# DavidPetrus/ood_object_detection

Measured on AMD Instinct MI355X. Metric: images/sec, tf_efficientdet_d0 640px bf16 inference + OOD score (DetBenchPredict end-to-end), higher is better.
Workload: dtype bf16; 1 GPU; tf_efficientdet_d0 640x640 batch=64/GPU C=90, DetBenchPredict: backbone+BiFPN+heads+OOD energy/max-logit+top-k(5000)+decode+hard NMS; global_batch=64, parallelism=image-sharded dp1, no collective, weights=seeded reference init, randomised BN stats, class bias 0, launch=hipgraph, images_in_flight=192

## Files before the change

### include/effdet_hip.h

```cpp
#ifndef EFFDET_HIP_H
#define EFFDET_HIP_H

#ifdef __cplusplus
extern "C" {
#endif

#define EFFDET_F32 0
#define EFFDET_BF16 1
#define EFFDET_BF16X2 2
#define EFFDET_PAD_SYMMETRIC (1 << 24)

int effdet_abi_version(void);
const char* effdet_last_error(void);
int effdet_device_error(int clear);


int effdet_stem_conv(void* stream, int in_dtype, int out_dtype, const void* X, const float* Wt,
                     const float* scale, const float* shift, void* Y, int B, int H, int W, int Cout);

int effdet_stem_dw_fused(void* stream, int in_dtype, int dtype, const void* X, const void* Wk,
                         const float* s1, const float* t1, const float* taps, const float* s2, const float* t2,
                         void* Y, float* pool_partial, int B, int H, int W, int C);
int effdet_stem_dw_parts(int dtype, int H, int W, int C);
#define EFFDET_STEM_DW_PLAN_INTS 13
int effdet_stem_dw_plan_describe(int dtype, int in_dtype, int H, int W, int C, int* out, int n);

int effdet_resize_pad_u8(void* stream, const unsigned char* src, int h, int w, unsigned char* dst, int S, int sw, int sh,
                         const int* bounds_x, const int* coef_x, int ksize_x,
                         const int* bounds_y, const int* coef_y, int ksize_y,
                         const int* fill_rgb, unsigned char* workspace);
int effdet_normalize_u8(void* stream, int out_dtype, const unsigned char* X, const float* mean, const float* stdv,
                        void* Y, int B, int C, long long hw);

typedef struct EffdetResampleDesc {
    const unsigned char* src;
    int h, w;
    int flip_h, flip_v;
    int cx0, cy0, cw, ch;
    int filter;
    int sw, sh;
    int ox, oy;
    int reserved;
} EffdetResampleDesc;
int effdet_resample_batch_u8(void* stream, const EffdetResampleDesc* desc, const EffdetResampleDesc* desc_host, int B,
                             unsigned char* dst, long long dst_image_stride, int S, const int* fill_rgb);

typedef struct EffdetBoxParams {
    float img_w, img_h;
    int flip_h, flip_v;
    float pre_y, pre_x, scale, post_y, post_x, clip_h, clip_w;
    int reserved;
} EffdetBoxParams;
int effdet_transform_boxes(void* stream, const float* boxes, const long long* classes, const EffdetBoxParams* params,
                           int B, int Mmax, float* out_boxes, long long* out_classes, int* counts, unsigned char* valid);
int effdet_stem_conv_u8(void* stream, int out_dtype, const unsigned char* X, const float* mean, const float* stdv,
                        const float* Wt, const float* scale, const float* shift, void* Y, int B, int H, int W, int Cout);
int effdet_stem_dw_fused_u8(void* stream, int dtype, const unsigned char* X, const float* mean, const float* stdv,
                            const void* Wk, const float* s1, const float* t1, const float* taps, const float* s2, const float* t2,
                            void* Y, float* pool_partial, int B, int H, int W, int C);

int effdet_pw_gemm_bn_act(void* stream, int dtype, const void* A, long long M, int K, const void* W, int N,
                          const float* scale, const float* shift, int act, const void* residual,
                          const float* gate, int rows_per_image,
                          void* C, long long c_image_stride, long long ldc);
int effdet_pw_gemm_group(void* stream, int dtype, int n, const void* const* A, const long long* M, const int* K,
                         const void* const* W, const int* N, const float* const* scale, const float* const* shift,
                         int act, void* const* C);
#define EFFDET_PW_GEMM_PLAN_INTS 13
int effdet_pw_gemm_plan_describe(int dtype, long long M, int K, int N, int rows_per_image, int gated, int has_residual,
                                 long long ldc, long long c_image_stride, int aligned, int group, int* out, int n);
int effdet_pw_gemm_group_plan_describe(int dtype, int n_problems, const long long* M, const int* K, const int* N, int aligned,
                                       int which, int* out, int n);

int effdet_dwconv_bn_act(void* stream, int dtype, const void* X, void* Y, const float* Wt,
                         const float* scale, const float* shift, int act, float* pool_partial,
                         int B, int H, int W, int C, int k, int stride);
int effdet_dwconv_blocks_per_image(int Ho, int Wo, int C);
#define EFFDET_DWCONV_PLAN_INTS 10
int effdet_dwconv_plan_describe(int dtype, int H, int W, int C, int k, int stride, int pooled, int* out, int n);

int effdet_mbconv_expand_dw(void* stream, int dtype, const void* X, void* Y, const void* W1,
                            const float* s1, const float* t1, const float* taps,
                            const float* s2, const float* t2, float* pool_partial,
                            int B, int H, int W, int Cin, int mid, int k, int stride);
int effdet_mbconv_tiles_per_image(int dtype, int H, int W, int Cin, int mid, int k, int stride);
int effdet_mbconv_expand_dw_gated(void* stream, int dtype, const void* X, const float* in_gate, void* Y, const void* W1,
                                  const float* s1, const float* t1, const float* taps,
                                  const float* s2, const float* t2, float* pool_partial,
                                  int B, int H, int W, int Cin, int mid, int k, int stride);
int effdet_mbconv_gated_tiles_per_image(int dtype, int H, int W, int Cin, int mid, int k, int stride);
#define EFFDET_MBCONV_PLAN_INTS 17
int effdet_mbconv_plan_describe(int dtype, int H, int W, int Cin, int mid, int k, int stride, int gated, int* out, int n);

int effdet_se_gate(void* stream, const float* partial, int nblk, int hw, const float* W1, const float* b1,
                   const float* W2t, const float* b2, float* gate, int B, int C, int R);


int effdet_maxpool_same(void* stream, int dtype, const void* X, long long x_image_stride,
                        void* Y, long long y_image_stride, int B, int H, int W, int C);

int effdet_sepconv_fused(void* stream, int dtype, int B, int nlevels, const int* level_hw, int n_in,
                         const void* const* in_ptr, const long long* in_image_stride, const int* in_hw,
                         const int* in_mode, int fuse_mode, const float* fuse_w, float fuse_den, int pre_act,
                         const float* dw_w, const void* pw_w, const float* scale, const float* shift,
                         const int* affine_row, int post_act, int F, int N,
                         void* const* out_ptr, const long long* out_image_stride,
                         int ood_classes, int num_anchors, float* ood_energy, float* ood_maxlogit,
                         long long ood_image_stride, const long long* ood_level_off);
#define EFFDET_SEPCONV_PLAN_INTS 18
int effdet_sepconv_plan_describe(int dtype, int nlevels, const int* level_hw, int n_in, int F, int N, int ood_classes,
                                 int num_anchors, int has_scale, int post_act, int aligned, int* out, int n);

int effdet_sepconv_meta(void* stream, int dtype, int B, int nlevels, const int* level_hw,
                        const void* const* in_ptr, const long long* in_image_stride,
                        const float* in_scale, const float* in_shift, const int* in_affine_row, int pre_act,
                        const float* dw_w, const void* pw_w, const float* bias, int F, int N,
                        void* const* out_ptr, const long long* out_image_stride,
                        float* stat_partial, void* const* dw_out, const long long* dw_out_image_stride);
int effdet_sepconv_tiles(int dtype, int nlevels, const int* level_hw, int* level_tile_begin);
int effdet_bn_batch_stats(void* stream, int dtype, const float* partial, int B, int nlevels, const int* level_hw, int N,
                          const float* weight, const float* bias, const int* param_row, float eps,
                          float* out_scale, float* out_shift);


long long effdet_topk_workspace_bytes(int B, long long n_anchors);
// ... 466 lines not shown
```

### ood_object_detection_amd/_lib.py

```python
import ctypes
import os
import subprocess

_HERE = os.path.dirname(os.path.abspath(__file__))
LIB_PATH = os.path.join(_HERE, 'libeffdet_hip.so')
CSRC = os.path.join(_HERE, 'csrc')

_lib = None

LABEL_PAD = -2 ** 63

c_void_p, c_int, c_ll, c_float, c_double = ctypes.c_void_p, ctypes.c_int, ctypes.c_longlong, ctypes.c_float, ctypes.c_double
P = ctypes.POINTER

SIGNATURES = {
    'effdet_abi_version': (c_int, []),
    'effdet_last_error': (ctypes.c_char_p, []),
    'effdet_device_error': (c_int, [c_int]),
    'effdet_stem_conv': (c_int, [c_void_p, c_int, c_int, c_void_p, c_void_p, c_void_p, c_void_p, c_void_p,
                                 c_int, c_int, c_int, c_int]),
    'effdet_stem_dw_fused': (c_int, [c_void_p, c_int, c_int, c_void_p, c_void_p, c_void_p, c_void_p, c_void_p, c_void_p,
                                     c_void_p, c_void_p, c_void_p, c_int, c_int, c_int, c_int]),
    'effdet_resize_pad_u8': (c_int, [c_void_p, c_void_p, c_int, c_int, c_void_p, c_int, c_int, c_int, c_void_p, c_void_p, c_int,
                                     c_void_p, c_void_p, c_int, c_void_p, c_void_p]),
    'effdet_resample_batch_u8': (c_int, [c_void_p, c_void_p, c_void_p, c_int, c_void_p, c_ll, c_int, c_void_p]),
    'effdet_transform_boxes': (c_int, [c_void_p, c_void_p, c_void_p, c_void_p, c_int, c_int, c_void_p, c_void_p, c_void_p, c_void_p]),
    'effdet_normalize_u8': (c_int, [c_void_p, c_int, c_void_p, c_void_p, c_void_p, c_void_p, c_int, c_int, c_ll]),
    'effdet_stem_conv_u8': (c_int, [c_void_p, c_int, c_void_p, c_void_p, c_void_p, c_void_p, c_void_p, c_void_p, c_void_p,
                                    c_int, c_int, c_int, c_int]),
    'effdet_stem_dw_fused_u8': (c_int, [c_void_p, c_int, c_void_p, c_void_p, c_void_p, c_void_p, c_void_p, c_void_p, c_void_p,
                                        c_void_p, c_void_p, c_void_p, c_void_p, c_int, c_int, c_int, c_int]),
    'effdet_stem_dw_parts': (c_int, [c_int, c_int, c_int, c_int]),
    'effdet_stem_dw_plan_describe': (c_int, [c_int, c_int, c_int, c_int, c_int, P(c_int), c_int]),
    'effdet_pw_gemm_bn_act': (c_int, [c_void_p, c_int, c_void_p, c_ll, c_int, c_void_p, c_int, c_void_p, c_void_p,
                                      c_int, c_void_p, c_void_p, c_int, c_void_p, c_ll, c_ll]),
    'effdet_pw_gemm_group': (c_int, [c_void_p, c_int, c_int, P(c_void_p), P(c_ll), P(c_int), P(c_void_p), P(c_int), P(c_void_p),
                                     P(c_void_p), c_int, P(c_void_p)]),
    'effdet_dwconv_bn_act': (c_int, [c_void_p, c_int, c_void_p, c_void_p, c_void_p, c_void_p, c_void_p, c_int,
                                     c_void_p, c_int, c_int, c_int, c_int, c_int, c_int]),
    'effdet_dwconv_blocks_per_image': (c_int, [c_int, c_int, c_int]),
    'effdet_dwconv_plan_describe': (c_int, [c_int, c_int, c_int, c_int, c_int, c_int, c_int, P(c_int), c_int]),
    'effdet_pw_gemm_plan_describe': (c_int, [c_int, c_ll, c_int, c_int, c_int, c_int, c_int, c_ll, c_ll, c_int, c_int, P(c_int), c_int]),
    'effdet_pw_gemm_group_plan_describe': (c_int, [c_int, c_int, P(c_ll), P(c_int), P(c_int), c_int, c_int, P(c_int), c_int]),
    'effdet_mbconv_gated_tiles_per_image': (c_int, [c_int, c_int, c_int, c_int, c_int, c_int, c_int]),
    'effdet_mbconv_expand_dw_gated': (c_int, [c_void_p, c_int, c_void_p, c_void_p, c_void_p, c_void_p, c_void_p, c_void_p, c_void_p,
                                              c_void_p, c_void_p, c_void_p, c_int, c_int, c_int, c_int, c_int, c_int, c_int]),
    'effdet_mbconv_expand_dw': (c_int, [c_void_p, c_int, c_void_p, c_void_p, c_void_p, c_void_p, c_void_p, c_void_p,
                                        c_void_p, c_void_p, c_void_p, c_int, c_int, c_int, c_int, c_int, c_int, c_int]),
    'effdet_mbconv_tiles_per_image': (c_int, [c_int, c_int, c_int, c_int, c_int, c_int, c_int]),
    'effdet_mbconv_plan_describe': (c_int, [c_int, c_int, c_int, c_int, c_int, c_int, c_int, c_int, P(c_int), c_int]),
    'effdet_se_gate': (c_int, [c_void_p, c_void_p, c_int, c_int, c_void_p, c_void_p, c_void_p, c_void_p,
                               c_void_p, c_int, c_int, c_int]),
    'effdet_maxpool_same': (c_int, [c_void_p, c_int, c_void_p, c_ll, c_void_p, c_ll, c_int, c_int, c_int, c_int]),
    'effdet_sepconv_fused': (c_int, [c_void_p, c_int, c_int, c_int, P(c_int), c_int,
                                     P(c_void_p), P(c_ll), P(c_int), P(c_int), c_int, P(c_float), c_float, c_int,
                                     c_void_p, c_void_p, c_void_p, c_void_p, P(c_int), c_int, c_int, c_int,
                                     P(c_void_p), P(c_ll), c_int, c_int, c_void_p, c_void_p, c_ll, P(c_ll)]),
    'effdet_sepconv_plan_describe': (c_int, [c_int, c_int, P(c_int), c_int, c_int, c_int, c_int, c_int, c_int, c_int, c_int, P(c_int), c_int]),
    'effdet_weighted_median': (c_int, [c_void_p, c_void_p, c_void_p, c_int, c_int, c_void_p, c_void_p]),
    'effdet_sqnorm_workspace_floats': (c_ll, []),
    'effdet_sqnorm': (c_int, [c_void_p, c_void_p, c_ll, c_void_p, c_void_p, c_int]),
    'effdet_adam_clip_step': (c_int, [c_void_p, c_void_p, c_void_p, c_void_p, c_void_p, c_ll, c_float, c_float, c_float, c_float,
                                      c_int, c_float, c_void_p]),
    'effdet_adam_clip_step_dev': (c_int, [c_void_p, c_void_p, c_void_p, c_void_p, c_void_p, c_ll, c_float, c_float, c_float, c_float,
                                          c_void_p, c_float, c_void_p]),
    'effdet_group_piece_floats': (c_ll, []),
    'effdet_group_norms': (c_int, [c_void_p, c_void_p, c_ll, c_void_p, c_int, c_int, c_void_p, c_int, c_void_p, c_int, c_void_p, c_int,
                                   c_void_p, c_void_p]),
    'effdet_group_step': (c_int, [c_void_p, c_int, c_void_p, c_void_p, c_void_p, c_void_p, c_ll, c_void_p, c_int, c_int, c_void_p, c_int,
                                  c_void_p, c_int, c_void_p, c_int, c_void_p, c_void_p, c_void_p, c_void_p]),
    'effdet_novelty_score': (c_int, [c_void_p, c_void_p, c_void_p, c_void_p, c_int, c_int, c_int, c_float, c_float, c_int,
                                     c_void_p, c_void_p, c_void_p]),
    'effdet_ood_image_score': (c_int, [c_void_p, c_void_p, c_int, c_ll, c_void_p]),
    'effdet_auroc_counts': (c_int, [c_void_p, c_void_p, c_void_p, c_int, c_int, c_void_p]),
    'effdet_ood_eval_workspace_bytes': (c_ll, [c_ll, c_ll]),
    'effdet_ood_eval_sort_tile': (c_int, []),
    'effdet_ood_eval_sorted_offset': (c_ll, [c_ll, c_ll, c_int]),
    'effdet_ood_eval_append': (c_int, [c_void_p, c_void_p, c_ll, c_ll, c_int, c_int, c_void_p, c_int, c_void_p, c_ll, c_ll, c_float,
                                       c_int, c_void_p, c_ll, c_void_p, c_void_p, c_ll]),
    'effdet_ood_eval_sort': (c_int, [c_void_p, c_void_p, c_ll, c_void_p, c_ll, c_void_p, c_void_p, c_ll]),
    'effdet_ood_eval_metrics': (c_int, [c_void_p, c_ll, c_ll, c_void_p, c_void_p, c_ll, c_double, c_void_p]),
    'effdet_feature_ood_workspace_bytes': (c_ll, [c_ll, c_int]),
    'effdet_feature_ood_fit': (c_int, [c_void_p, c_int, c_int, P(c_void_p), P(c_ll), P(c_ll), P(c_ll), P(c_ll), c_int, c_int, c_int, c_int,
                                       c_ll, c_void_p, c_void_p, c_int, c_ll, c_ll, c_ll, c_void_p, c_int, c_void_p, c_void_p, c_void_p,
                                       c_void_p, c_ll]),
    'effdet_feature_ood_score': (c_int, [c_void_p, c_int, c_int, P(c_void_p), P(c_ll), P(c_ll), P(c_ll), P(c_ll), c_int, c_int, c_int,
                                         c_int, c_ll, c_void_p, c_void_p, c_int, c_void_p, c_void_p, c_void_p, c_void_p, c_void_p,
                                         c_void_p, c_void_p, c_void_p]),
    'effdet_feature_knn_workspace_bytes': (c_ll, [c_ll, c_int, c_int, c_int]),
    'effdet_feature_knn_append': (c_int, [c_void_p, c_int, c_int, P(c_void_p), P(c_ll), P(c_ll), P(c_ll), P(c_ll), c_int, c_int, c_int, c_int,
                                          c_ll, c_void_p, c_void_p, c_int, c_ll, c_ll, c_ll, c_void_p, c_int, c_int, c_ll, c_ll, c_void_p,
                                          c_void_p, c_void_p, c_void_p, c_void_p, c_ll]),
    'effdet_feature_knn_score': (c_int, [c_void_p, c_int, c_int, P(c_void_p), P(c_ll), P(c_ll), P(c_ll), P(c_ll), c_int, c_int, c_int,
                                         c_ll, c_void_p, c_void_p, c_int, c_int, c_int, c_int, c_ll, c_void_p, c_void_p, c_void_p,
                                         c_void_p, c_void_p, c_void_p, c_void_p, c_ll]),
    'effdet_feature_subspace_score': (c_int, [c_void_p, c_int, c_int, P(c_void_p), P(c_ll), P(c_ll), P(c_ll), P(c_ll), c_int, c_int, c_int,
# ... 278 lines not shown
```

### ood_object_detection_amd/csrc/pw_gemm.hip

```cpp
#include "common.h"

namespace {

struct PwArgs {
    const void* A; long long M; int K;
    const void* W; int N;
    const float* scale; const float* shift; int act;
    const void* res;
    const float* gate; int rows_per_image;
    void* C; long long c_image_stride; long long ldc;
    int tiles_per_image, n_tiles, vec_ok;
};

template <int V> struct PwInt { static constexpr int value = V; };

constexpr int PW_PIX = 128;

template <typename T, int BN> struct PwGeom {
    static constexpr int KCH = IsPair<T>::value ? 1 : 2;
    static constexpr int ROWB = KCH * OpGeom<T>::CHUNK + 16;
    static constexpr int W_BYTES = BN * ROWB;
    static constexpr int LDS_BYTES = 2 * W_BYTES;
    __host__ __device__ static inline int chunks(int K) { return (K + OpGeom<T>::KPC - 1) / OpGeom<T>::KPC; }
    __host__ __device__ static inline int stages(int K) { return (chunks(K) + KCH - 1) / KCH; }
};

template <typename T, int BN, int PT, int NTH, bool GATED>
DEV void pw_gemm_body(const PwArgs& p, const int bid) {
    constexpr bool PAIR = IsPair<T>::value;
    constexpr int KCH = PwGeom<T, BN>::KCH;
    constexpr int EPC = VecTraits<T>::EPC;
    constexpr int KPC = OpGeom<T>::KPC;
    constexpr int PB = OpGeom<T>::PIECE, CB = OpGeom<T>::CHUNK;
    constexpr int NT = BN / 16, NP = NT / 2;
    static_assert(NT % 2 == 0, "tile pairs");
    constexpr int PF = 2;
    constexpr int ROWB = PwGeom<T, BN>::ROWB;
    constexpr int W_BYTES = PwGeom<T, BN>::W_BYTES;
    static_assert(ROWB == KCH * CB + 16, "one stage of K + 16 pad");
    __shared__ __attribute__((aligned(16))) char lds[PwGeom<T, BN>::LDS_BYTES];
    extern __shared__ __attribute__((aligned(16))) float gate_lds[];

    const int tid = threadIdx.x, lane = tid & 63, wave = tid >> 6;
    const int frow = lane & 15, fpiece = lane >> 4;
    const int K = p.K, N = p.N;
    const int nt = bid % p.n_tiles;
    const int mt = bid / p.n_tiles;
    const int img = mt / p.tiles_per_image;
    const int pix0 = (mt - img * p.tiles_per_image) * PW_PIX;
    const int n0 = nt * BN;
    const int n_count = (N - n0) < BN ? (N - n0) : BN;
    const long long pitch = (long long)K * (long long)sizeof(T);
    const int nst = PwGeom<T, BN>::stages(K);
// ... 277 lines not shown
        default: return EFFDET_EINVAL;
    }
#undef PW_LAUNCH
#undef PW_LAUNCH_G
#undef PW_FORM
    return plan ? EFFDET_OK : effdet_check_launch();
}

int pw_single(hipStream_t st, int dtype, PwArgs& a, PwPlan* plan) {
    if (!a.A || !a.W || !a.C || !a.shift || a.M <= 0 || a.K <= 0 || a.N <= 0) return EFFDET_EINVAL;
    if (a.K % 8 != 0 || a.M > 0x7fffffffLL) return EFFDET_EINVAL;
    if (a.act < 0 || a.act > 2) return EFFDET_EINVAL;
    if (a.rows_per_image <= 0) a.rows_per_image = (int)a.M;
    if ((a.M % a.rows_per_image) != 0) return EFFDET_EINVAL;
    if (a.ldc <= 0) a.ldc = a.N;
    if (a.c_image_stride <= 0) a.c_image_stride = (long long)a.rows_per_image * a.ldc;
    if (dtype == 0) return launch_pw<float>(st, a, plan);
    if (dtype == 1) return launch_pw<bf16_t>(st, a, plan);
    if (dtype == 2) {
        if (a.N % 8 || a.ldc % 8 || a.c_image_stride % 8 || reinterpret_cast<uintptr_t>(a.A) % 32 || reinterpret_cast<uintptr_t>(a.W) % 32 ||
            reinterpret_cast<uintptr_t>(a.C) % 32 || (a.res && reinterpret_cast<uintptr_t>(a.res) % 32)) return EFFDET_EINVAL;
        return launch_pw<bf16p_t>(st, a, plan);
    }
    return EFFDET_EINVAL;
}

int pw_group(hipStream_t st, int dtype, int n, const void* const* A, const long long* M, const int* K, const void* const* W, const int* N,
             const float* const* scale, const float* const* shift, int act, void* const* C, PwPlan* plan, int which) {
    if (n < 1 || n > PW_GROUP_MAX || !A || !M || !K || !W || !N || !scale || !shift || !C || act < 0 || act > 2) return EFFDET_EINVAL;
    if (which < 0 || which >= n) return EFFDET_EINVAL;
    PwGroupArgs g;
    g.n = n;
    for (int i = 0; i < n; ++i) {
        if (!A[i] || !W[i] || !C[i] || !shift[i] || M[i] <= 0 || M[i] > 0x7fffffffLL || K[i] <= 0 || K[i] % 8 || N[i] <= 0) return EFFDET_EINVAL;
        g.p[i] = PwArgs{A[i], M[i], K[i], W[i], N[i], scale[i], shift[i], act, nullptr, nullptr, (int)M[i], C[i], M[i] * N[i], N[i], 0, 0, 0};
    }
    if (dtype == 0) return launch_pw_group<float>(st, g, plan, which);
    if (dtype == 1) return launch_pw_group<bf16_t>(st, g, plan, which);
    if (dtype == 2) {
        for (int i = 0; i < n; ++i)
            if (N[i] % 8 || reinterpret_cast<uintptr_t>(A[i]) % 32 || reinterpret_cast<uintptr_t>(W[i]) % 32 || reinterpret_cast<uintptr_t>(C[i]) % 32)
                return EFFDET_EINVAL;
        return launch_pw_group<bf16p_t>(st, g, plan, which);
    }
    return EFFDET_EINVAL;
}

int pw_plan_out(const PwPlan& plan, int* out, int n) {
    const int m = n < EFFDET_PW_GEMM_PLAN_INTS ? n : EFFDET_PW_GEMM_PLAN_INTS;
    for (int i = 0; i < m; ++i) out[i] = plan.v[i];
    return m;
}

}

extern "C" int effdet_pw_gemm_bn_act(void* stream, int dtype,
                                     const void* A, long long M, int K,
                                     const void* W, int N,
                                     const float* scale, const float* shift, int act,
                                     const void* residual,
                                     const float* gate, int rows_per_image,
                                     void* C, long long c_image_stride, long long ldc) {
    EFFDET_ENTER();
    PwArgs a{A, M, K, W, N, scale, shift, act, residual, gate, rows_per_image, C, c_image_stride, ldc, 0, 0, 0};
    return pw_single(reinterpret_cast<hipStream_t>(stream), dtype, a, nullptr);
}

extern "C" int effdet_pw_gemm_group(void* stream, int dtype, int n, const void* const* A, const long long* M, const int* K,
                                    const void* const* W, const int* N, const float* const* scale, const float* const* shift,
                                    int act, void* const* C) {
    EFFDET_ENTER();
    return pw_group(reinterpret_cast<hipStream_t>(stream), dtype, n, A, M, K, W, N, scale, shift, act, C, nullptr, 0);
}

extern "C" int effdet_pw_gemm_group_plan_describe(int dtype, int n_problems, const long long* M, const int* K, const int* N, int aligned,
                                                  int which, int* out, int n) {
    if (!out || n <= 0 || !M || !K || !N || n_problems < 1 || n_problems > PW_GROUP_MAX) return EFFDET_EINVAL;
    (void)take_pad_flag(dtype);
    static const float present = 1.0f;
    void* const at = reinterpret_cast<void*>(aligned ? (uintptr_t)64 : (uintptr_t)4);
    const void* ptr[PW_GROUP_MAX]; void* cptr[PW_GROUP_MAX]; const float* fptr[PW_GROUP_MAX];
    for (int i = 0; i < PW_GROUP_MAX; ++i) { ptr[i] = at; cptr[i] = at; fptr[i] = &present; }
    PwPlan plan{};
    const int rc = pw_group(nullptr, dtype, n_problems, ptr, M, K, ptr, N, fptr, fptr, 0, cptr, &plan, which);
    return rc != EFFDET_OK ? rc : pw_plan_out(plan, out, n);
}

extern "C" int effdet_pw_gemm_plan_describe(int dtype, long long M, int K, int N, int rows_per_image, int gated, int has_residual,
                                            long long ldc, long long c_image_stride, int aligned, int group, int* out, int n) {
    if (!out || n <= 0) return EFFDET_EINVAL;
    if (group) {
        if (gated || has_residual || (ldc > 0 && ldc != N) || (c_image_stride > 0 && c_image_stride != M * N)) return EFFDET_EINVAL;
        if (rows_per_image > 0 && rows_per_image != M) return EFFDET_EINVAL;
        return effdet_pw_gemm_group_plan_describe(dtype, 1, &M, &K, &N, aligned, 0, out, n);
    }
    (void)take_pad_flag(dtype);
    static const float present = 1.0f;
    void* const at = reinterpret_cast<void*>(aligned ? (uintptr_t)64 : (uintptr_t)4);
    PwArgs a{at, M, K, at, N, &present, &present, 0, has_residual ? at : nullptr, gated ? &present : nullptr, rows_per_image, at,
             c_image_stride, ldc, 0, 0, 0};
    PwPlan plan{};
    const int rc = pw_single(nullptr, dtype, a, &plan);
    return rc != EFFDET_OK ? rc : pw_plan_out(plan, out, n);
}
```

### ood_object_detection_amd/engine.py

```python
import ctypes
import math

import torch

from . import _lib
from . import pairfmt

_DT = {torch.float32: 0, torch.bfloat16: 1}
_PAIR = 2
_PAD_SYMMETRIC = 1 << 24


def _same_out(n, s):
    return (n + s - 1) // s


def _arr(ctype, values):
    return (ctype * len(values))(*values)


class Engine(object):
    def __init__(self, model, B, image_size, ood_out=None):
        cfg = model.config
        self._ood_out = ood_out
        self.wtoken = model.weights_token()
        p0 = model.backbone.conv_stem.weight
        if p0.device.type != 'cuda':
            raise RuntimeError('the EfficientDet HIP path needs the model on a GPU (cuda:N); there is no CPU fallback')
        if p0.dtype not in _DT:
            raise RuntimeError('supported parameter dtypes: float32, bfloat16 (got %s)' % p0.dtype)
        self.lib = _lib.load()
        self.device, self.dtype, self.dt = p0.device, p0.dtype, _DT[p0.dtype]
        self.mode = getattr(model, 'compute_mode', 'native') or 'native'
        self.keep_class_tower = bool(getattr(model, 'keep_class_tower', False))
        if self.mode not in ('native', 'accurate'):
            raise ValueError("compute_mode must be 'native' or 'accurate' (got %r)" % (self.mode,))
        self.pair = self.mode == 'accurate'
        self.bb_pad = _PAD_SYMMETRIC if getattr(model.backbone, 'pad_type', 'same') == '' else 0
        self.fpn_pad = _PAD_SYMMETRIC if cfg.pad_type == '' else 0
        if self.pair:
            if p0.dtype != torch.float32:
                raise RuntimeError("compute_mode='accurate' splits float32 master weights into two bf16 terms: it needs a float32 model")
            self.dt = _PAIR
        self.B, self.image_size = B, tuple(image_size)
        self.cfg = cfg
        self.F = cfg.fpn_channels
        self.C = cfg.num_classes
        self.A = model.num_anchors
        self.L = cfg.num_levels
        self._keep = []
        self.input_mean = tuple(getattr(model, 'input_mean', (0.485, 0.456, 0.406)))
        self.input_std = tuple(getattr(model, 'input_std', (0.229, 0.224, 0.225)))
        self.pyr_es = torch.empty(0, dtype=self.dtype).element_size()
        H, W = self.image_size
        if cfg.fpn_channels > 288:
            raise NotImplementedError('BiFPN / head width %d: the fused separable-conv kernel keeps a tile of all channels in LDS and is '
                                      'built for widths up to 288 (tf_efficientdet_d0 ... d5); d6 / d7 are not built' % cfg.fpn_channels)
        if H % (2 ** cfg.max_level) or W % (2 ** cfg.max_level):
            raise ValueError('image size must be divisible by 2**max_level (reference: effdet/anchors.py:229-230)')
        with torch.no_grad():
            self._build_backbone(model.backbone, H, W)
            self._build_fpn(model.fpn)
            self._build_heads(model)

    def matches(self, model):
        p0 = model.backbone.conv_stem.weight
        return p0.device == self.device and p0.dtype == self.dtype and model.config.num_classes == self.C and \
            (getattr(model, 'compute_mode', 'native') or 'native') == self.mode and \
            bool(getattr(model, 'keep_class_tower', False)) == self.keep_class_tower

    def _new(self, *shape, dtype=None):
        t = torch.empty(*shape, dtype=dtype or self.dtype, device=self.device)
        self._keep.append(t)
        return t

    def _f32(self, t):
        t = t.detach().to(device=self.device, dtype=torch.float32).contiguous()
        self._keep.append(t)
        return t

    def _w(self, t):
        if self.pair:
            t = pairfmt.encode(t.detach().to(device=self.device, dtype=torch.float32))
        else:
            t = t.detach().to(device=self.device, dtype=self.dtype).contiguous()
        self._keep.append(t)
        return t

    def _act_in(self, t):
        return pairfmt.encode(t.float()) if self.pair else t

    def _act_out(self, t):
        return pairfmt.decode(t) if self.pair else t

    def _fold(self, bn, conv_bias=None):
        w, b = bn.weight.detach().float(), bn.bias.detach().float()
        m, v = bn.running_mean.detach().float(), bn.running_var.detach().float()
        scale = w / torch.sqrt(v + bn.eps)
        shift = b - m * scale
        if conv_bias is not None:
            shift = shift + conv_bias.detach().float() * scale
        return scale, shift

    @staticmethod
    def _dw_taps(w):
        k = w.shape[-1]
        return w.detach().float().permute(2, 3, 0, 1).reshape(k * k, w.shape[0])

    def _run(self, plan):
        st = torch.cuda.current_stream(self.device).cuda_stream
        for fn, args, what, _meta in plan:
            rc = fn(st, *args)
            if rc != 0:
                _lib.check(rc, what)

    def _gemm_meta(self, M, K, N, residual=False, gate=False):
        es = self.pyr_es
        b = (M * K + M * N + N * K) * es + (M * N * es if residual else 0) + (self.B * K * 4 if gate else 0)
        return dict(kind='pw_gemm', bytes=b, flops=2 * M * K * N)

    def profile(self, reps=5):
        st = torch.cuda.current_stream(self.device)
        out = []
        for plan in (self._bb_plan, self._fpn_plan, self._cls_plan, self._box_plan):
            for fn, args, what, meta in plan:
                e0, e1 = torch.cuda.Event(enable_timing=True), torch.cuda.Event(enable_timing=True)
                fn(st.cuda_stream, *args)
                e0.record(st)
                for _ in range(reps):
                    fn(st.cuda_stream, *args)
                e1.record(st)
                e1.synchronize()
                out.append((what, meta['kind'], meta['bytes'], meta['flops'], e0.elapsed_time(e1) / reps))
        return out

    def _build_backbone(self, bb, H, W):
        lib, B, dt = self.lib, self.B, self.dt
        dtp = dt | self.bb_pad
        stem_c, stages = bb.arch
        plan = []
        Hs, Ws = _same_out(H, 2), _same_out(W, 2)
        stem_parts = lib.effdet_stem_dw_parts(dtp, H, W, stem_c)
        io_max, mid_max, part_max, exp_max = B * Hs * Ws * stem_c, 0, 0, 0
        forms = []
        h, w = Hs, Ws
        for blocks in stages:
            forms.append([])
            for b in blocks:
                ho, wo = _same_out(h, b['s']), _same_out(w, b['s'])
                mid_max = max(mid_max, B * ho * wo * b['mid'])
                dw_parts = lib.effdet_dwconv_blocks_per_image(ho, wo, b['mid'])
                fused, rows = False, None
                if b['type'] == 'ir':
                    nblk = lib.effdet_mbconv_tiles_per_image(dtp, h, w, b['cin'], b['mid'], b['k'], b['s'])
                    fused = nblk > 0
                    if not fused:
                        nblk = dw_parts
                        exp_max = max(exp_max, B * h * w * b['mid'])
                else:
                    nblk = dw_parts
                    rows = max(nblk, stem_parts)
                if nblk <= 0:
                    raise NotImplementedError('block geometry (mid=%d) is outside the built range' % b['mid'])
                forms[-1].append((fused, nblk))
                part_max = max(part_max, B * (rows or nblk) * b['mid'])
                io_max = max(io_max, B * ho * wo * b['cout'])
                h, w = ho, wo
        ping = [self._new(io_max), self._new(io_max)]
        dbuf = self._new(max(mid_max, 1))
        b00, b10 = stages[0][0], (stages[1][0] if len(stages) > 1 else None)
        self._compose01 = bool(len(stages[0]) == 1 and b10 is not None and b00['type'] == 'ds' and not b00['residual']
                               and b10['type'] == 'ir' and not b10['residual'] and b00['mid'] % 8 == 0)
# ... 77 lines not shown
                        fused, nblk = forms[si][bi]
                        mid_buf = dbuf
                        if fused:
                            plan.append((lib.effdet_mbconv_expand_dw,
                                         (dtp, cur.data_ptr(), dbuf.data_ptr(), w1.data_ptr(), s1.data_ptr(), t1.data_ptr(),
                                          taps.data_ptr(), s2.data_ptr(), t2.data_ptr(), partial.data_ptr(),
                                          B, h, w, b['cin'], b['mid'], b['k'], b['s']), what + '.conv_pw+conv_dw',
                                         dict(kind='mbconv', bytes=B * (h * w * b['cin'] + ho * wo * b['mid']) * es + b['mid'] * b['cin'] * es,
                                              flops=2 * B * (h * w * b['cin'] * b['mid'] + b['k'] * b['k'] * ho * wo * b['mid']))))
                        else:
                            plan.append((lib.effdet_pw_gemm_bn_act,
                                         (dt, cur.data_ptr(), B * h * w, b['cin'], w1.data_ptr(), b['mid'], s1.data_ptr(),
                                          t1.data_ptr(), 1, None, None, 0, ebuf.data_ptr(), 0, 0), what + '.conv_pw',
                                         self._gemm_meta(B * h * w, b['cin'], b['mid'])))
                            plan.append((lib.effdet_dwconv_bn_act,
                                         (dtp, ebuf.data_ptr(), dbuf.data_ptr(), taps.data_ptr(), s2.data_ptr(), t2.data_ptr(), 1,
                                          partial.data_ptr(), B, h, w, b['mid'], b['k'], b['s']), what + '.conv_dw',
                                         dict(kind='dwconv', bytes=B * (h * w + ho * wo) * b['mid'] * es,
                                              flops=2 * b['k'] * b['k'] * B * ho * wo * b['mid'])))
                    pw_out, bn_out = m.conv_pwl, m.bn3
                elif si == 0 and bi == 0 and self._fuse_stem:
                    nblk = stem_parts
                    pw_out, bn_out = m.conv_pw, m.bn2
                    mid_buf = dbuf
                else:
                    s2, t2 = self._fold(m.bn1)
                    taps = self._f32(self._dw_taps(m.conv_dw.weight))
                    s2, t2 = self._f32(s2), self._f32(t2)
                    nblk = forms[si][bi][1]
                    plan.append((lib.effdet_dwconv_bn_act,
                                 (dtp, cur.data_ptr(), dbuf.data_ptr(), taps.data_ptr(), s2.data_ptr(), t2.data_ptr(), 1,
                                  partial.data_ptr(), B, h, w, b['mid'], b['k'], b['s']), what + '.conv_dw',
                                 dict(kind='dwconv', bytes=B * (h * w + ho * wo) * b['mid'] * es,
                                      flops=2 * b['k'] * b['k'] * B * ho * wo * b['mid'])))
                    pw_out, bn_out = m.conv_pw, m.bn2
                    mid_buf = dbuf
                W1 = self._f32(m.se.conv_reduce.weight.reshape(b['se'], b['mid']))
                b1 = self._f32(m.se.conv_reduce.bias)
                W2 = self._f32(m.se.conv_expand.weight.reshape(b['mid'], b['se']).t())
                b2 = self._f32(m.se.conv_expand.bias)
                plan.append((lib.effdet_se_gate,
                             (partial.data_ptr(), nblk, ho * wo, W1.data_ptr(), b1.data_ptr(), W2.data_ptr(), b2.data_ptr(),
                              gate.data_ptr(), B, b['mid'], b['se']), what + '.se',
                             dict(kind='se_gate', bytes=B * (nblk + 1) * b['mid'] * 4 + 8 * b['mid'] * b['se'],
                                  flops=4 * B * b['mid'] * b['se'])))
                s3, t3 = self._fold(bn_out)
                if si == 0 and bi == 0 and self._compose01 and self._fuse_stem:
                    composed = (pw_out.weight.detach().reshape(b['cout'], b['mid']).to(device=self.device, dtype=torch.float32),
                                s3.to(device=self.device, dtype=torch.float32), t3.to(device=self.device, dtype=torch.float32), b['mid'])
                    cur, h, w = None, ho, wo
                    continue
                w3 = self._w(pw_out.weight.reshape(b['cout'], b['mid']))
                s3, t3 = self._f32(s3), self._f32(t3)
                plan.append((lib.effdet_pw_gemm_bn_act,
                             (dt, mid_buf.data_ptr(), B * ho * wo, b['mid'], w3.data_ptr(), b['cout'], s3.data_ptr(),
                              t3.data_ptr(), 0, cur.data_ptr() if b['residual'] else None, gate.data_ptr(), ho * wo,
                              out.data_ptr(), 0, 0), what + '.conv_pwl',
                             self._gemm_meta(B * ho * wo, b['mid'], b['cout'], residual=b['residual'], gate=True)))
                cur, h, w = out, ho, wo
        self._bb_plan = plan
        self.feat_hw = [(f.shape[1], f.shape[2]) for f in self.feats]

    def run_backbone(self, x, ret=True):
        if tuple(x.shape) != self.x_shape:
            raise ValueError('engine was prepared for input %s, got %s' % (self.x_shape, tuple(x.shape)))
        if x.device != self.device or (x.dtype not in _DT and x.dtype != torch.uint8):
            raise RuntimeError('input must be a float32/bfloat16 (normalised) or uint8 (raw) tensor on %s' % (self.device,))
        if self.pair and x.dtype == torch.bfloat16:
            x = x.float()
        x = x.contiguous()
        self._stem_call(x)
        self._run(self._bb_plan)
        return [self._act_out(f).permute(0, 3, 1, 2) for f in self.feats] if ret else None

    def _stem_call(self, x):
        st = torch.cuda.current_stream(self.device).cuda_stream
        if x.dtype == torch.uint8:
            import ctypes
            mean = (ctypes.c_float * 3)(*[255.0 * v for v in self.input_mean])
            std = (ctypes.c_float * 3)(*[255.0 * v for v in self.input_std])
            if self._fuse_stem:
                wk, s, t, taps0, s2, t2, dbuf, partial, H, W, c = self._stem
                _lib.check(self.lib.effdet_stem_dw_fused_u8(st, self.dt | self.bb_pad, x.data_ptr(), mean, std, wk.data_ptr(), s.data_ptr(),
                                                            t.data_ptr(), taps0.data_ptr(), s2.data_ptr(), t2.data_ptr(),
                                                            dbuf.data_ptr(), partial.data_ptr(), self.B, H, W, c),
                           'backbone.conv_stem+blocks.0.0.conv_dw (uint8)')
            else:
                wt, s, t, out, H, W, c = self._stem
                _lib.check(self.lib.effdet_stem_conv_u8(st, self.dt | self.bb_pad, x.data_ptr(), mean, std, wt.data_ptr(), s.data_ptr(),
                                                        t.data_ptr(), out.data_ptr(), self.B, H, W, c), 'backbone.conv_stem (uint8)')
            return
        if self._fuse_stem:
            wk, s, t, taps0, s2, t2, dbuf, partial, H, W, c = self._stem
            _lib.check(self.lib.effdet_stem_dw_fused(st, _DT[x.dtype], self.dt | self.bb_pad, x.data_ptr(), wk.data_ptr(), s.data_ptr(),
                                                     t.data_ptr(), taps0.data_ptr(), s2.data_ptr(), t2.data_ptr(),
                                                     dbuf.data_ptr(), partial.data_ptr(), self.B, H, W, c),
                       'backbone.conv_stem+blocks.0.0.conv_dw')
        else:
            wt, s, t, out, H, W, c = self._stem
            _lib.check(self.lib.effdet_stem_conv(st, _DT[x.dtype], self.dt | self.bb_pad, x.data_ptr(), wt.data_ptr(), s.data_ptr(),
                                                 t.data_ptr(), out.data_ptr(), self.B, H, W, c), 'backbone.conv_stem')

    def _build_fpn(self, fpn):
        lib, B, dt, F, cfg = self.lib, self.B, self.dt, self.F, self.cfg
        plan = []
        lateral = []
        in_info = fpn.in_feature_info
        nbb = len(in_info)
        hw = list(self.feat_hw)
        while len(hw) < self.L:
            hw.append((_same_out(hw[-1][0], 2), _same_out(hw[-1][1], 2)))
# ... 277 lines not shown
```

Baseline: 17220 images/sec.

## Add LDS-resident weight kernel for gated MBConv project convs

Adds a new project-conv GEMM kernel that stages each weight slice into LDS once per workgroup, with the SE gate pre-multiplied into the weights, then streams the activation tiles of one image through MFMA against the resident weights. Grid mapping is XCD-aware. A host-side byte-model heuristic picks this kernel over the tiled GEMM only when its modelled traffic is well below the tiled one. The aim is to cut repeated weight and activation reads in the backbone's projection convs. The cost is a large LDS footprint (up to 160KB), which lowers occupancy.

```diff
diff --git a/include/effdet_hip.h b/include/effdet_hip.h
--- a/include/effdet_hip.h
+++ b/include/effdet_hip.h
@@ -71,6 +71,13 @@
                                  long long ldc, long long c_image_stride, int aligned, int group, int* out, int n);
 int effdet_pw_gemm_group_plan_describe(int dtype, int n_problems, const long long* M, const int* K, const int* N, int aligned,
                                        int which, int* out, int n);
+
+int effdet_project_conv_resident(void* stream, int dtype, const void* A, long long M, int K, const void* W, int N,
+                                 const float* scale, const float* shift, const void* residual,
+                                 const float* gate, int rows_per_image, void* C, long long c_image_stride, long long ldc);
+#define EFFDET_PROJECT_CONV_PLAN_INTS 13
+int effdet_project_conv_resident_plan_describe(int dtype, long long M, int K, int N, int rows_per_image, int gated, int has_residual,
+                                               long long ldc, long long c_image_stride, int aligned, int* out, int n);
 
 int effdet_dwconv_bn_act(void* stream, int dtype, const void* X, void* Y, const float* Wt,
                          const float* scale, const float* shift, int act, float* pool_partial,
diff --git a/ood_object_detection_amd/_lib.py b/ood_object_detection_amd/_lib.py
--- a/ood_object_detection_amd/_lib.py
+++ b/ood_object_detection_amd/_lib.py
@@ -42,6 +42,10 @@
     'effdet_dwconv_plan_describe': (c_int, [c_int, c_int, c_int, c_int, c_int, c_int, c_int, P(c_int), c_int]),
     'effdet_pw_gemm_plan_describe': (c_int, [c_int, c_ll, c_int, c_int, c_int, c_int, c_int, c_ll, c_ll, c_int, c_int, P(c_int), c_int]),
     'effdet_pw_gemm_group_plan_describe': (c_int, [c_int, c_int, P(c_ll), P(c_int), P(c_int), c_int, c_int, P(c_int), c_int]),
+    'effdet_project_conv_resident': (c_int, [c_void_p, c_int, c_void_p, c_ll, c_int, c_void_p, c_int, c_void_p, c_void_p,
+                                             c_void_p, c_void_p, c_int, c_void_p, c_ll, c_ll]),
+    'effdet_project_conv_resident_plan_describe': (c_int, [c_int, c_ll, c_int, c_int, c_int, c_int, c_int, c_ll, c_ll, c_int,
+                                                           P(c_int), c_int]),
     'effdet_mbconv_gated_tiles_per_image': (c_int, [c_int, c_int, c_int, c_int, c_int, c_int, c_int]),
     'effdet_mbconv_expand_dw_gated': (c_int, [c_void_p, c_int, c_void_p, c_void_p, c_void_p, c_void_p, c_void_p, c_void_p, c_void_p,
                                               c_void_p, c_void_p, c_void_p, c_int, c_int, c_int, c_int, c_int, c_int, c_int]),
diff --git a/ood_object_detection_amd/csrc/pw_gemm.hip b/ood_object_detection_amd/csrc/pw_gemm.hip
--- a/ood_object_detection_amd/csrc/pw_gemm.hip
+++ b/ood_object_detection_amd/csrc/pw_gemm.hip
@@ -1,4 +1,5 @@
 #include "common.h"
+#include <utility>
 
 namespace {
 
@@ -382,6 +383,279 @@
     return m;
 }
 
+struct PwResArgs {
+    const void* A; const void* W; const float* scale; const float* shift; const void* res; const float* gate; void* C;
+    long long c_image_stride, ldc;
+    int K, N, rows_per_image, images;
+    int nsl, slice, parts, tiles;
+};
+
+constexpr int PWR_NTH = 512;
+constexpr int PWR_PTMAX = 4;
+constexpr int PWR_RUN_MAX = PWR_PTMAX * (PWR_NTH / 64);
+constexpr int PWR_LDS_BUDGET = 160 * 1024;
+constexpr int PWR_PAD = 32;
+constexpr int PWR_CUS = 256;
+
+template <typename F, int... I> DEV void pw_static_for(F&& f, std::integer_sequence<int, I...>) { (f(IntC<I>{}), ...); }
+
+template <int BN, int NTH>
+__global__ __launch_bounds__(NTH) void pw_resident_kernel(PwResArgs p) {
+    typedef bf16_t T;
+    constexpr int NT = BN / 16, NP = NT / 2, NW = NTH / 64;
+    extern __shared__ __attribute__((aligned(16))) char res_lds[];
+    const int tid = threadIdx.x, lane = tid & 63, wave = __builtin_amdgcn_readfirstlane(tid >> 6);
+    const int frow = lane & 15, fpiece = lane >> 4;
+    const int K = p.K, N = p.N;
+    const int xcd = blockIdx.x & 7, rr = blockIdx.x >> 3;
+    const int per_image = p.nsl * p.parts;
+    const int img = (rr / per_image) * 8 + xcd;
+    if (img >= p.images) return;
+    const int q = rr % per_image;
+    const int sl = q % p.nsl, part = q / p.nsl;
+    const int n0 = sl * p.slice;
+    const int n_count = (N - n0) < p.slice ? (N - n0) : p.slice;
+    const int t0 = (int)((long long)part * p.tiles / p.parts), t1 = (int)((long long)(part + 1) * p.tiles / p.parts);
+    const long long pitch = (long long)K * 2;
+    const int rowb = K * 2 + PWR_PAD;
+    const int nch = K >> 5;
+    float* gate_lds = reinterpret_cast<float*>(res_lds);
+    char* wl = res_lds + K * 4;
+    const int G = n_count >> 5, g4 = ((n_count & 31) >> 3) * 4;
+
+    auto stage_w = [&]() __attribute__((always_inline)) {
+        const float* gate = p.gate + (long long)img * K;
+        for (int k = tid * 4; k < K; k += NTH * 4) *reinterpret_cast<f32x4*>(gate_lds + k) = *reinterpret_cast<const f32x4*>(gate + k);
+        __syncthreads();
+        const char* Wb = reinterpret_cast<const char*>(p.W) + (long long)n0 * pitch;
+        const int ppr = K >> 3;
+        const int total = n_count * ppr;
+        const int dco = NTH / ppr, dpc = NTH % ppr;
+        int co = tid / ppr, pc = tid % ppr;
+        constexpr int U = 8;
+        for (int base = 0; base < total; base += NTH * U) {
+            u32x4 w[U];
+            int cou[U], pcu[U];
+#pragma unroll
+            for (int u = 0; u < U; ++u) {
+                cou[u] = co; pcu[u] = pc;
+                const bool ok = co < n_count;
+                w[u] = *reinterpret_cast<const u32x4*>(Wb + (long long)(ok ? co : 0) * pitch + (ok ? pc : 0) * 16);
+                co += dco; pc += dpc;
+                if (pc >= ppr) { pc -= ppr; ++co; }
+            }
+#pragma unroll
+            for (int u = 0; u < U; ++u) {
+                if (cou[u] < n_count) {
+                    const f32x4 g0 = *reinterpret_cast<const f32x4*>(gate_lds + pcu[u] * 8);
+                    const f32x4 g1 = *reinterpret_cast<const f32x4*>(gate_lds + pcu[u] * 8 + 4);
+                    bf16x8 x = __builtin_bit_cast(bf16x8, w[u]);
+#pragma unroll
+                    for (int e = 0; e < 8; ++e) x[e] = (bf16_t)((float)x[e] * (e < 4 ? g0[e] : g1[e - 4]));
+                    const int c = cou[u], J = c >> 5, half = (c >> 2) & 1, r = 4 * ((c >> 3) & 3) + (c & 3);
+                    const int row = J < G ? 16 * (2 * J + half) + r : 32 * G + half * g4 + r;
+                    *reinterpret_cast<u32x4*>(wl + row * rowb + pcu[u] * 16) = __builtin_bit_cast(u32x4, x);
+                }
+            }
+        }
+        __syncthreads();
+    };
+
+    auto body = [&](auto PTC) __attribute__((always_inline)) {
+        constexpr int PT = decltype(PTC)::value;
+        constexpr int D = PT == 1 ? 8 : PT == 2 ? 6 : (PT == 4 && NT == 8) ? 3 : 4;
+        const char* arow[PT];
+        int pix[PT];
+        bool pix_ok[PT];
+#pragma unroll
+        for (int i = 0; i < PT; ++i) {
+            pix[i] = (t0 + wave + NW * i) * 16 + frow;
+            pix_ok[i] = pix[i] < p.rows_per_image;
+            const long long m = (long long)img * p.rows_per_image + (pix_ok[i] ? pix[i] : 0);
+            arow[i] = reinterpret_cast<const char*>(p.A) + m * pitch + fpiece * 16;
+        }
+        Frag<T> areg[D][PT];
+        auto a_load = [&](int c, int slot) __attribute__((always_inline)) {
+#pragma unroll
+            for (int i = 0; i < PT; ++i) areg[slot][i] = ld_frag<T>(arow[i] + c * 64);
+        };
+        f32x4 acc[PT][NT];
+#pragma unroll
+        for (int i = 0; i < PT; ++i)
+#pragma unroll
+            for (int j = 0; j < NT; ++j) acc[i][j] = f32x4{0.f, 0.f, 0.f, 0.f};
+#pragma unroll
+        for (int s = 0; s < D - 1; ++s) a_load(s < nch ? s : nch - 1, s);
+        stage_w();
+
+        int woff[NT];
+#pragma unroll
+        for (int j = 0; j < NT; ++j) {
+            const int J = j >> 1;
+            int row = 16 * j + frow;
+            if (J >= G) row = (J == G && g4 > 0) ? 32 * G + (j & 1) * g4 + (frow < g4 ? frow : g4 - 1) : 0;
+            woff[j] = row * rowb + fpiece * 16;
+        }
+        auto step = [&](int c, auto UC, auto LOAD) __attribute__((always_inline)) {
+            constexpr int u = decltype(UC)::value;
+            if constexpr (decltype(LOAD)::value) a_load(c + D - 1 < nch ? c + D - 1 : nch - 1, (u + D - 1) % D);
+#pragma unroll
+            for (int j = 0; j < NT; ++j) {
+                const Frag<T> wf = ld_frag<T>(wl + woff[j] + c * 64);
+#pragma unroll
+                for (int i = 0; i < PT; ++i) mma_chunk(wf, areg[u][i], acc[i][j]);
+            }
+        };
+        int c = 0;
+        for (; c + D <= nch; c += D) pw_static_for([&](auto UC) { step(c + decltype(UC)::value, UC, IntC<1>{}); }, std::make_integer_sequence<int, D>{});
+        pw_static_for([&](auto UC) { if (c + decltype(UC)::value < nch) step(c + decltype(UC)::value, UC, IntC<0>{}); },
+                      std::make_integer_sequence<int, D - 1>{});
+
+        T* Cb = reinterpret_cast<T*>(p.C) + (long long)img * p.c_image_stride;
+        const T* Rb = reinterpret_cast<const T*>(p.res);
+        const int njp = (n_count + 31) / 32;
+#pragma unroll
+        for (int J = 0; J < NP; ++J) {
+            if (J < njp) {
+                const int cb = 32 * J + 8 * fpiece;
+                if (n_count - cb > 0) {
+                    float sc[8], sh[8];
+#pragma unroll
+                    for (int e = 0; e < 8; ++e) {
+                        sc[e] = p.scale ? p.scale[n0 + cb + e] : 1.0f;
+                        sh[e] = p.shift[n0 + cb + e];
+                    }
+#pragma unroll
+                    for (int i = 0; i < PT; ++i) {
+                        if (!pix_ok[i]) continue;
+                        float v[8];
+#pragma unroll
+                        for (int r = 0; r < 4; ++r) {
+                            v[r] = fmaf(acc[i][2 * J][r], sc[r], sh[r]);
+                            v[4 + r] = fmaf(acc[i][2 * J + 1][r], sc[4 + r], sh[4 + r]);
+                        }
+                        if (Rb != nullptr) {
+                            const F8 rv = load8<T>(Rb + ((long long)img * p.rows_per_image + pix[i]) * N + n0 + cb);
+#pragma unroll
+                            for (int e = 0; e < 8; ++e) v[e] += rv.v[e];
+                        }
+                        F8 o;
+#pragma unroll
+                        for (int e = 0; e < 8; ++e) o.v[e] = v[e];
+                        store8<T>(Cb + (long long)pix[i] * p.ldc + n0 + cb, o);
+                    }
+                }
+            }
+        }
+    };
+
+    const int ntiles = t1 - t0;
+    const int cnt = wave < ntiles ? (ntiles - wave + NW - 1) / NW : 0;
+    switch (cnt) {
+        case 0: stage_w(); break;
+        case 1: body(IntC<1>{}); break;
+        case 2: body(IntC<2>{}); break;
+        case 3: body(IntC<3>{}); break;
+        default: body(IntC<4>{}); break;
+    }
+}
+
+struct PwResGeom { int bn, nsl, slice, parts, tiles, lds, run_min, run_max; long long grid; };
+
+int pw_res_geometry(long long images, int rows, int K, int N, PwResGeom& g) {
+    const int rowb = K * 2 + PWR_PAD;
+    const long long room = (long long)PWR_LDS_BUDGET - (long long)K * 4;
+    if (room < 32LL * rowb) return EFFDET_EINVAL;
+    int fit = (int)(room / rowb);
+    if (fit > 128) fit = 128;
+    if (N <= fit) { g.nsl = 1; g.slice = N; }
+    else {
+        const int cap = fit / 32 * 32;
+        g.nsl = (N + cap - 1) / cap;
+        g.slice = ((N + g.nsl - 1) / g.nsl + 31) / 32 * 32;
+        if (g.slice > cap) { g.slice = cap; g.nsl = (N + cap - 1) / cap; }
+    }
+    g.bn = (g.slice + 31) / 32 * 32;
+    g.lds = K * 4 + g.slice * rowb;
+    g.tiles = (rows + 15) / 16;
+    const int pmin = (g.tiles + PWR_RUN_MAX - 1) / PWR_RUN_MAX;
+    const int pmax = g.tiles;
+    long long best = -1;
+    g.parts = pmin;
+    for (int P = pmin; P <= pmax && P < pmin + 4 * PWR_CUS; ++P) {
+        const long long wgs = images * g.nsl * P;
+        const long long rounds = (wgs + PWR_CUS - 1) / PWR_CUS;
+        const long long cost = rounds * ((long long)((g.tiles + P - 1) / P) * 16 * K * 2 + (long long)g.slice * K * 2);
+        if (best < 0 || cost < best) { best = cost; g.parts = P; }
+    }
+    g.run_min = g.tiles / g.parts;
+    g.run_max = (g.tiles + g.parts - 1) / g.parts;
+    g.grid = (images + 7) / 8 * 8 * g.nsl * g.parts;
+    if (g.grid > 0x7fffffffLL) return EFFDET_EINVAL;
+    return EFFDET_OK;
+}
+
+int pw_resident(hipStream_t st, int dtype, PwResArgs& a, long long M, int* plan) {
+    if (dtype != 1 || !a.A || !a.W || !a.C || !a.shift || !a.gate || M <= 0 || a.K <= 0 || a.N <= 0) return EFFDET_EINVAL;
+    if (a.K % 32 != 0 || M > 0x7fffffffLL) return EFFDET_EINVAL;
+    if (a.rows_per_image <= 0) a.rows_per_image = (int)M;
+    if ((M % a.rows_per_image) != 0) return EFFDET_EINVAL;
+    if (a.ldc <= 0) a.ldc = a.N;
+    if (a.c_image_stride <= 0) a.c_image_stride = (long long)a.rows_per_image * a.ldc;
+    if (a.N % 8 != 0 || a.ldc % 8 != 0 || a.c_image_stride % 8 != 0 || a.ldc < a.N || reinterpret_cast<uintptr_t>(a.C) % 16 != 0 ||
+        reinterpret_cast<uintptr_t>(a.A) % 16 != 0 || reinterpret_cast<uintptr_t>(a.W) % 16 != 0 ||
+        (a.res != nullptr && reinterpret_cast<uintptr_t>(a.res) % 16 != 0)) return EFFDET_EINVAL;
+    a.images = (int)(M / a.rows_per_image);
+    PwResGeom g;
+    const int rc = pw_res_geometry(a.images, a.rows_per_image, a.K, a.N, g);
+    if (rc) return rc;
+    a.nsl = g.nsl; a.slice = g.slice; a.parts = g.parts; a.tiles = g.tiles;
+    if (plan) {
+        const int v[EFFDET_PROJECT_CONV_PLAN_INTS] = {g.bn, PWR_NTH, g.nsl, g.slice, g.parts, g.tiles, (int)g.grid, g.lds, g.run_min, g.run_max,
+                                                      a.K / 32, a.images * g.nsl * g.parts, PWR_CUS};
+        for (int i = 0; i < EFFDET_PROJECT_CONV_PLAN_INTS; ++i) plan[i] = v[i];
+        return EFFDET_OK;
+    }
+    void (*kern)(PwResArgs) = nullptr;
+    switch (g.bn) {
+        case 32:  kern = pw_resident_kernel<32, PWR_NTH>; break;
+        case 64:  kern = pw_resident_kernel<64, PWR_NTH>; break;
+        case 96:  kern = pw_resident_kernel<96, PWR_NTH>; break;
+        case 128: kern = pw_resident_kernel<128, PWR_NTH>; break;
+        default: return EFFDET_EINVAL;
+    }
+    if (g.lds > 64 * 1024) {
+        if (hipFuncSetAttribute(reinterpret_cast<const void*>(kern), hipFuncAttributeMaxDynamicSharedMemorySize, PWR_LDS_BUDGET) != hipSuccess)
+            return EFFDET_ELAUNCH;
+    }
+    hipLaunchKernelGGL(kern, dim3((unsigned)g.grid), dim3(PWR_NTH), (size_t)g.lds, st, a);
+    return effdet_check_launch();
+}
+
+}
+
+extern "C" int effdet_project_conv_resident(void* stream, int dtype, const void* A, long long M, int K, const void* W, int N,
+                                            const float* scale, const float* shift, const void* residual,
+                                            const float* gate, int rows_per_image, void* C, long long c_image_stride, long long ldc) {
+    EFFDET_ENTER();
+    PwResArgs a{A, W, scale, shift, residual, gate, C, c_image_stride, ldc, K, N, rows_per_image, 0, 0, 0, 0, 0};
+    return pw_resident(reinterpret_cast<hipStream_t>(stream), dtype, a, M, nullptr);
+}
+
+extern "C" int effdet_project_conv_resident_plan_describe(int dtype, long long M, int K, int N, int rows_per_image, int gated,
+                                                          int has_residual, long long ldc, long long c_image_stride, int aligned,
+                                                          int* out, int n) {
+    if (!out || n <= 0) return EFFDET_EINVAL;
+    static const float present = 1.0f;
+    void* const at = reinterpret_cast<void*>(aligned ? (uintptr_t)64 : (uintptr_t)4);
+    PwResArgs a{at, at, &present, &present, has_residual ? at : nullptr, gated ? &present : nullptr, at, c_image_stride, ldc, K, N,
+                rows_per_image, 0, 0, 0, 0, 0};
+    int plan[EFFDET_PROJECT_CONV_PLAN_INTS];
+    const int rc = pw_resident(nullptr, dtype, a, M, plan);
+    if (rc != EFFDET_OK) return rc;
+    const int m = n < EFFDET_PROJECT_CONV_PLAN_INTS ? n : EFFDET_PROJECT_CONV_PLAN_INTS;
+    for (int i = 0; i < m; ++i) out[i] = plan[i];
+    return m;
 }
 
 extern "C" int effdet_pw_gemm_bn_act(void* stream, int dtype,
diff --git a/ood_object_detection_amd/engine.py b/ood_object_detection_amd/engine.py
--- a/ood_object_detection_amd/engine.py
+++ b/ood_object_detection_amd/engine.py
@@ -1,5 +1,6 @@
 import ctypes
 import math
+import os
 
 import torch
 
@@ -36,6 +37,10 @@
         if self.mode not in ('native', 'accurate'):
             raise ValueError("compute_mode must be 'native' or 'accurate' (got %r)" % (self.mode,))
         self.pair = self.mode == 'accurate'
+        self._resident = os.environ.get('EFFDET_PROJECT_CONV_RESIDENT', 'auto') or 'auto'
+        if self._resident not in ('auto', '0', '1'):
+            raise ValueError("EFFDET_PROJECT_CONV_RESIDENT must be 'auto', '0' or '1' (got %r)" % (self._resident,))
+        self.resident_launches = []
         self.bb_pad = _PAD_SYMMETRIC if getattr(model.backbone, 'pad_type', 'same') == '' else 0
         self.fpn_pad = _PAD_SYMMETRIC if cfg.pad_type == '' else 0
         if self.pair:
@@ -118,6 +123,33 @@
         es = self.pyr_es
         b = (M * K + M * N + N * K) * es + (M * N * es if residual else 0) + (self.B * K * 4 if gate else 0)
         return dict(kind='pw_gemm', bytes=b, flops=2 * M * K * N)
+
+    RESIDENT_GAIN = 0.7
+    RESIDENT_L2_REREAD = 0.5
+
+    @staticmethod
+    def project_conv_bytes_per_pixel(lib, M, rows, K, N, residual):
+        out = (ctypes.c_int * 13)()
+        n = lib.effdet_pw_gemm_plan_describe(1, M, K, N, rows, 1, int(bool(residual)), 0, 0, 1, 0, out, 13)
+        if n < 8:
+            raise RuntimeError('effdet_pw_gemm_plan_describe refused a project conv (%d)' % n)
+        bn, tiles_pi, n_tiles = out[0], out[4], out[5]
+        tiled = 2.0 * K * n_tiles + 2.0 * K * bn * tiles_pi / rows
+        n = lib.effdet_project_conv_resident_plan_describe(1, M, K, N, rows, 1, int(bool(residual)), 0, 0, 1, out, 13)
+        if n < 13:
+            return tiled, None
+        nsl, slice_, parts, work, slots = out[2], out[3], out[4], out[11], out[12]
+        fill = work / float((work + slots - 1) // slots * slots)
+        return tiled, (2.0 * K * (1.0 + Engine.RESIDENT_L2_REREAD * (nsl - 1)) + 2.0 * K * slice_ * parts / rows) / fill
+
+    @classmethod
+    def project_conv_resident(cls, lib, M, rows, K, N, residual, switch='auto'):
+        if switch == '0':
+            return False
+        tiled, resident = cls.project_conv_bytes_per_pixel(lib, M, rows, K, N, residual)
+        if resident is None:
+            return False
+        return switch == '1' or resident <= cls.RESIDENT_GAIN * tiled
 
     def profile(self, reps=5):
         st = torch.cuda.current_stream(self.device)
@@ -301,11 +333,19 @@
                     continue
                 w3 = self._w(pw_out.weight.reshape(b['cout'], b['mid']))
                 s3, t3 = self._f32(s3), self._f32(t3)
-                plan.append((lib.effdet_pw_gemm_bn_act,
-                             (dt, mid_buf.data_ptr(), B * ho * wo, b['mid'], w3.data_ptr(), b['cout'], s3.data_ptr(),
-                              t3.data_ptr(), 0, cur.data_ptr() if b['residual'] else None, gate.data_ptr(), ho * wo,
-                              out.data_ptr(), 0, 0), what + '.conv_pwl',
-                             self._gemm_meta(B * ho * wo, b['mid'], b['cout'], residual=b['residual'], gate=True)))
+                res_ptr = cur.data_ptr() if b['residual'] else None
+                if dt == 1 and self.project_conv_resident(lib, B * ho * wo, ho * wo, b['mid'], b['cout'], b['residual'], self._resident):
+                    self.resident_launches.append(what + '.conv_pwl')
+                    plan.append((lib.effdet_project_conv_resident,
+                                 (dt, mid_buf.data_ptr(), B * ho * wo, b['mid'], w3.data_ptr(), b['cout'], s3.data_ptr(),
+                                  t3.data_ptr(), res_ptr, gate.data_ptr(), ho * wo, out.data_ptr(), 0, 0), what + '.conv_pwl',
+                                 self._gemm_meta(B * ho * wo, b['mid'], b['cout'], residual=b['residual'], gate=True)))
+                else:
+                    plan.append((lib.effdet_pw_gemm_bn_act,
+                                 (dt, mid_buf.data_ptr(), B * ho * wo, b['mid'], w3.data_ptr(), b['cout'], s3.data_ptr(),
+                                  t3.data_ptr(), 0, res_ptr, gate.data_ptr(), ho * wo,
+                                  out.data_ptr(), 0, 0), what + '.conv_pwl',
+                                 self._gemm_meta(B * ho * wo, b['mid'], b['cout'], residual=b['residual'], gate=True)))
                 cur, h, w = out, ho, wo
         self._bb_plan = plan
         self.feat_hw = [(f.shape[1], f.shape[2]) for f in self.feats]
```

Result: slower. 16930 images/sec (-1.7%).
